# taohan10200/CRA5

Hardware: AMD Instinct MI355X
Metric: ERA5 frames/s (721x1440x268) encode+decode (higher is better)
Workload: dtype f32 (3xf16-split MFMA, fp32 accumulate)

## Files before the change

cra5_amd/csrc/attention_split_f16.hip:

```cpp
#include <hip/hip_runtime.h>
#include <math.h>
#include <stdlib.h>

#include "../../include/cra5_amd.h"
#include "split.h"

CRA5_RANGE_TU(attn)

typedef float f32x16 __attribute__((ext_vector_type(16)));
typedef _Float16 half8 __attribute__((ext_vector_type(8)));
typedef _Float16 half4 __attribute__((ext_vector_type(4)));
typedef __fp16 fp16x4 __attribute__((__vector_size__(4 * sizeof(__fp16))));
#if defined(__HIP_DEVICE_COMPILE__)
#define CRA5_TR_READ(P) \
  __builtin_bit_cast(half4, __builtin_amdgcn_ds_read_tr16_b64_v4f16((__attribute__((address_space(3))) fp16x4 *)(P)))
#else
#define CRA5_TR_READ(P) (*reinterpret_cast<const half4 *>(P))
#endif

namespace {

__device__ __forceinline__ int xcd_remap(int bid, int nb) {
  const int q = nb / 8, r = nb % 8;
  const int xcd = bid % 8, within = bid / 8;
  const int base = (xcd < r) ? xcd * (q + 1) : r * (q + 1) + (xcd - r) * q;
  return base + within;
}

struct WinGeom {
  int H, W, wh, ww, nwc;
};

__device__ __forceinline__ int token_of(const WinGeom &g, int wr, int wc, int t) {
  if (g.ww == g.W && g.wh == g.H) return t;
  const int r = t / g.ww, c = t - r * g.ww;
  const int gr = wr * g.wh + r, gc = wc * g.ww + c;
  return (gr < g.H && gc < g.W) ? gr * g.W + gc : -1;
}

#ifdef CRA5_ATTN_TRACE
__device__ unsigned long long g_attn_trace[6 * 8192];
#define CRA5_ATRACE(SLOT, VAL)                                                                          \
  if (threadIdx.x == 0 && atrace_idx < 8192) g_attn_trace[atrace_idx * 6 + (SLOT)] = (VAL);
#else
#define CRA5_ATRACE(SLOT, VAL)
#endif

constexpr int HD = 64;
constexpr int KS = 72;
constexpr int VS = 96;
constexpr int MAX_WIN_TOKENS = 1152;

struct BalArgs {
  int groups;
  int n_full;
  int n_wg_pass;
  int rem_tile0;
  int rem;
  int n_grp;
  int nkt;
  int maxp;
  float *ws;
};
__host__ __device__ __forceinline__ long bal_cut(long S, int G, int c) { return S * c / G; }
__host__ __device__ __forceinline__ int bal_piece_of(long S, int G, long s) {
  int c = (int)(s * G / S);
  if (c > G - 1) c = G - 1;
  while (c > 0 && bal_cut(S, G, c) > s) --c;
  while (c < G - 1 && bal_cut(S, G, c + 1) <= s) ++c;
  return c;
}
constexpr int WS_ROW = 68;

template <int NW, bool HI, bool GLOBAL, bool BAL = false, bool PLAIN = false>
__global__ __launch_bounds__(NW * 64, (NW >= 8 ? 1 : (NW == 4 ? 3 : 2))) void window_attention_split_kernel(
    const unsigned short *__restrict__ qkv, long ldq ,
    const unsigned short *__restrict__ pad_row, float *__restrict__ out, unsigned short *__restrict__ out_s,
    int Kp_out, int C, int heads, WinGeom g, int q_tiles , float scale, BalArgs bal) {
  static_assert(!BAL || GLOBAL, "the balanced schedule is for whole-grid launches");
  static_assert(!PLAIN || HI, "plain rows carry no lo plane");
  constexpr int NT = NW * 64;
  constexpr int PPR = PLAIN ? 8 : 16;
  constexpr int PIECES = 32 * PPR;
  constexpr int STG = (PIECES + NT - 1) / NT;

  constexpr int KPL = 32 * KS + 32;
  constexpr int VPL = 32 * VS;
  constexpr int KBUF = 2 * KPL, VBUF = 2 * VPL;
  __shared__ __attribute__((aligned(16))) unsigned short lds[2 * KBUF + 2 * VBUF];
  unsigned short *Ks = lds;
  unsigned short *Vt = lds + 2 * KBUF;
  constexpr int TAB = GLOBAL ? 1 : MAX_WIN_TOKENS;
  __shared__ long long tab[TAB];

  const int L = g.wh * g.ww;
  int head, win, n_seg = 1;
  int seg_tile0[2] = {0, 0}, seg_nact[2] = {NW, NW}, seg_j0[2] = {0, 0}, seg_j1[2] = {L / 32, L / 32}, seg_part[2] = {-1, -1};
  int seg_grp[2] = {0, 0};
  if (BAL) {
    const int pass = blockIdx.x / bal.n_wg_pass, w = blockIdx.x - pass * bal.n_wg_pass;
    int slot;
    if ((heads & 7) == 0 && (bal.n_wg_pass & 7) == 0) {
      const int xcd = w & 7, s_ = w >> 3;
      head = xcd * (heads >> 3) + s_ / bal.groups;
      slot = s_ % bal.groups;
    } else {
      head = w / bal.groups;
      slot = w % bal.groups;
    }
    win = 0;
    if (pass < bal.n_full) {
      seg_tile0[0] = (pass * bal.groups + slot) * NW;
    } else {
      const long S = (long)bal.n_grp * bal.nkt;
      const long s0 = bal_cut(S, bal.groups, slot), s1 = bal_cut(S, bal.groups, slot + 1);
      n_seg = 0;
      for (long s = s0; s < s1;) {
        const int gq = (int)(s / bal.nkt);
        const long e = min(s1, (long)(gq + 1) * bal.nkt);
        if (n_seg < 2) {
          seg_grp[n_seg] = gq;
          seg_tile0[n_seg] = bal.rem_tile0 + gq * NW;
          seg_nact[n_seg] = min(NW, bal.rem - gq * NW);
          seg_j0[n_seg] = (int)(s - (long)gq * bal.nkt);
          seg_j1[n_seg] = (int)(e - (long)gq * bal.nkt);
          seg_part[n_seg] = slot - bal_piece_of(S, bal.groups, (long)gq * bal.nkt);
          ++n_seg;
        }
        s = e;
      }
    }
  } else {
    const int pid = xcd_remap(blockIdx.x, gridDim.x);
    const int qt = pid % q_tiles;
    const int wh_id = pid / q_tiles;
    head = wh_id % heads;
    win = wh_id / heads;
    seg_tile0[0] = qt * NW;
  }
  const int wr = win / g.nwc, wc = win - wr * g.nwc;

  const int tid = threadIdx.x, lane = tid & 63, wave = tid >> 6;
  const int l31 = lane & 31, h = lane >> 5;
  const int hoff = head * HD;
  const long qoff = (PLAIN ? 1L : 2L) * hoff, koff = (PLAIN ? 1L : 2L) * (C + hoff), voff = (PLAIN ? 1L : 2L) * (2 * C + hoff);

  if (!GLOBAL) {
    const long long pad_delta = reinterpret_cast<const char *>(pad_row) - reinterpret_cast<const char *>(qkv);
    for (int t = tid; t < L; t += NT) {
      const int tok = token_of(g, wr, wc, t);
      tab[t] = (tok >= 0) ? (long long)tok * ldq * 2 : pad_delta;
    }
  }
  constexpr bool IDLE_SKIP = !GLOBAL || BAL;
  bool tab_ready = GLOBAL;
#pragma unroll 1
  for (int seg = 0; seg < n_seg; ++seg) {
  const int tile0 = seg_tile0[seg], n_active = seg_nact[seg], j0 = seg_j0[seg], j1 = seg_j1[seg];
#ifdef CRA5_ATTN_TRACE
  const int atrace_idx = GLOBAL ? 8192 : (int)blockIdx.x;
  const unsigned long long atrace_c0 = clock64();
#endif
  CRA5_ATRACE(0, wall_clock64());
  const int tq = (tile0 + wave) * 32 + l31;
  const int q_tok = (tq < L && wave < n_active) ? token_of(g, wr, wc, tq) : -1;
  const bool wave_active = __any(q_tok >= 0);
  if (!__syncthreads_or(wave_active ? 1 : 0)) continue;
  tab_ready = true;

  half8 qh[4], ql[4];
  {
    const unsigned short *qrow = ((q_tok >= 0) ? qkv + (size_t)q_tok * ldq : pad_row) + qoff;
#pragma unroll
    for (int s = 0; s < 4; ++s) {
      const int chunk = s >> 1, pp = 2 * (s & 1) + h;
      if (PLAIN) {
        qh[s] = *reinterpret_cast<const half8 *>(qrow + 16 * s + 8 * h);
        ql[s] = qh[s];
      } else {
        qh[s] = *reinterpret_cast<const half8 *>(qrow + chunk * 64 + pp * 8);
        ql[s] = *reinterpret_cast<const half8 *>(qrow + chunk * 64 + 32 + pp * 8);
      }
    }
  }
  const float cexp = scale * 1.44269504088896340736f;
  f32x16 negm;
#pragma unroll
  for (int r = 0; r < 16; ++r) negm[r] = 0.f;
  if (HI) {
#pragma unroll
    for (int s = 0; s < 4; ++s)
#pragma unroll
      for (int e = 0; e < 8; ++e) qh[s][e] = (_Float16)((float)qh[s][e] * cexp);
  }
  const float cmax = HI ? 1.0f : cexp;

  f32x16 o[2];
#pragma unroll
  for (int t = 0; t < 2; ++t)
#pragma unroll
    for (int r = 0; r < 16; ++r) o[t][r] = 0.f;
  float m_run = HI ? 0.f : -INFINITY, l_run = 0.f;

  const int n_tiles = j1 - j0;
  uint4 sk0 = make_uint4(0u, 0u, 0u, 0u), sk1 = sk0, sv0 = sk0, sv1 = sk0;
  static_assert(STG == 1 || STG == 2, "staging below is written out for one or two 16-byte pieces per thread");
  constexpr bool TWO = STG == 2;
  const int krow0 = min(tid / PPR, 31), krow1 = min((tid + NT) / PPR, 31);
  const long kcol = koff + (tid % PPR) * 8;
  const long vcol = voff + (tid % PPR) * 8;
  const unsigned short *kq0 = qkv + (size_t)(krow0 + 32 * j0) * ldq + kcol;
  const unsigned short *kq1 = qkv + (size_t)(krow1 + 32 * j0) * ldq + kcol;
  const unsigned short *vq0 = qkv + (size_t)(krow0 + 32 * j0) * ldq + vcol;
  const unsigned short *vq1 = qkv + (size_t)(krow1 + 32 * j0) * ldq + vcol;
  const long tile_step = 32 * ldq;
#define CRA5_ROW(JJ, ROW) \
  reinterpret_cast<const unsigned short *>(reinterpret_cast<const char *>(qkv) + tab[(JJ)*32 + (ROW)])
  const bool stage0 = (NT <= PIECES) || (tid < PIECES);
  const bool stage1 = TWO && (tid + NT < PIECES);
#define CRA5_K_LOAD(J)                                                                    \
  if (stage0) {                                                                           \
    if (GLOBAL) {                                                                         \
      sk0 = *reinterpret_cast<const uint4 *>(kq0);                                        \
      if (stage1) sk1 = *reinterpret_cast<const uint4 *>(kq1);                            \
      const long st_ = ((J) < n_tiles - 1) ? tile_step : 0;  \
      kq0 += st_;                                                                         \
      kq1 += st_;                                                                         \
    } else {                                                                              \
      const int jj_ = min((J), n_tiles - 1);                                              \
      sk0 = *reinterpret_cast<const uint4 *>(CRA5_ROW(jj_, krow0) + kcol);                \
      if (stage1) sk1 = *reinterpret_cast<const uint4 *>(CRA5_ROW(jj_, krow1) + kcol);    \
    }                                                                                     \
  }
#define CRA5_V_LOAD(J)                                                                    \
  if (stage0) {                                                                           \
    if (GLOBAL) {                                                                         \
      sv0 = *reinterpret_cast<const uint4 *>(vq0);                                        \
      if (stage1) sv1 = *reinterpret_cast<const uint4 *>(vq1);                            \
      const long st_ = ((J) < n_tiles - 1) ? tile_step : 0;                               \
      vq0 += st_;                                                                         \
      vq1 += st_;                                                                         \
    } else {                                                                              \
      const int jj_ = min((J), n_tiles - 1);                                              \
      sv0 = *reinterpret_cast<const uint4 *>(CRA5_ROW(jj_, krow0) + vcol);                \
      if (stage1) sv1 = *reinterpret_cast<const uint4 *>(CRA5_ROW(jj_, krow1) + vcol);    \
    }                                                                                     \
  }
#define CRA5_K_STORE1(P, BUF)                                                             \
  {                                                                                       \
    const int idx = tid + (P)*NT;                                                         \
    if (idx < PIECES) {                                                                   \
      const int row = idx / PPR, piece = idx % PPR;                                       \
      const int plane = PLAIN ? 0 : (piece >> 2) & 1, d0 = PLAIN ? 8 * piece : 32 * (piece >> 3) + 8 * (piece & 3); \
      *reinterpret_cast<uint4 *>(Ks + (BUF)*KBUF + plane * KPL + row * KS + d0) = sk##P;  \
    }                                                                                     \
  }
#define CRA5_K_STORE(BUF) { CRA5_K_STORE1(0, BUF) if (TWO) CRA5_K_STORE1(1, BUF) }
#define CRA5_V_STORE1(P, BUF)                                                             \
  {                                                                                       \
    const int idx = tid + (P)*NT;                                                         \
    if (idx < PIECES) {                                                                   \
      const int row = idx / PPR, piece = idx % PPR;                                       \
      const int plane = PLAIN ? 0 : (piece >> 2) & 1, d0 = PLAIN ? 8 * piece : 32 * (piece >> 3) + 8 * (piece & 3); \
      *reinterpret_cast<uint4 *>(Vt + (BUF)*VBUF + plane * VPL + row * VS + d0) = sv##P;  \
    }                                                                                     \
  }
#define CRA5_V_STORE(BUF) { CRA5_V_STORE1(0, BUF) if (TWO) CRA5_V_STORE1(1, BUF) }
#define CRA5_SCORES(DST, KB)                                                              \
  {                                                                                       \
    f32x16 acc_;                                                                          \
    _Pragma("unroll") for (int r = 0; r < 16; ++r) acc_[r] = 0.f;                         \
    _Pragma("unroll") for (int st = 0; st < 4; ++st) {                                    \
      const half8 kh = *reinterpret_cast<const half8 *>(k_base + (KB)*KBUF + 16 * st);     \
      const half8 kl = *reinterpret_cast<const half8 *>(k_base + (KB)*KBUF + KPL + 16 * st); \
      if (!HI) {                                                                          \
        acc_ = __builtin_amdgcn_mfma_f32_32x32x16_f16(kl, qh[st], acc_, 0, 0, 0);         \
        acc_ = __builtin_amdgcn_mfma_f32_32x32x16_f16(kh, ql[st], acc_, 0, 0, 0);         \
      }                                                                                   \
      if (HI && st == 0) {                                                                \
        CRA5_MFMA_FROM(acc_, kh, qh[0], negm);                                            \
      } else {                                                                            \
        acc_ = __builtin_amdgcn_mfma_f32_32x32x16_f16(kh, qh[st], acc_, 0, 0, 0);         \
      }                                                                                   \
    }                                                                                     \
    DST = acc_;                                                                           \
  }
#if defined(__HIP_DEVICE_COMPILE__)
#define CRA5_MFMA_FROM(D, A, B, C) \
  asm("s_nop 3\n\tv_mfma_f32_32x32x16_f16 %0, %1, %2, %3" : "=&v"(D) : "v"(A), "v"(B), "v"(C))
#else
#define CRA5_MFMA_FROM(D, A, B, C) (D) = (C)
#endif

  const unsigned short *k_base = Ks + l31 * KS + 8 * h;
  const unsigned short *v_base = Vt + (4 * h + ((lane & 15) >> 2)) * VS + 16 * ((lane >> 4) & 1) + 4 * (lane & 3);

#if defined(__HIP_DEVICE_COMPILE__)
#define CRA5_XHALF_MAX(X)                                                                 \
  ({                                                                                      \
    float a_ = (X), b_ = (X), r_;                                                         \
    asm("s_nop 1\n\tv_permlane32_swap_b32_e32 %0, %1\n\ts_nop 1\n\tv_max_f32_e32 %2, %0, %1" \
        : "+v"(a_), "+v"(b_), "=v"(r_));                                                  \
    r_;                                                                                   \
  })
#define CRA5_MAX2_VALU(A, B)                                                              \
  ({                                                                                      \
    float r_;                                                                             \
    asm("v_max_f32_e32 %0, %1, %2" : "=v"(r_) : "v"(A), "v"(B));                          \
    r_;                                                                                   \
  })
#else
#define CRA5_XHALF_MAX(X) (X)
#define CRA5_MAX2_VALU(A, B) fmaxf((A), (B))
#endif
#if !defined(__HIP_DEVICE_COMPILE__)
#define CRA5_TILE_MAX(S)                                                                  \
  ({                                                                                      \
    float m_ = fmaxf(fmaxf(fmaxf(S[0], S[1]), fmaxf(S[2], S[3])), fmaxf(fmaxf(S[4], S[5]), fmaxf(S[6], S[7]))); \
    float n_ = fmaxf(fmaxf(fmaxf(S[8], S[9]), fmaxf(S[10], S[11])), fmaxf(fmaxf(S[12], S[13]), fmaxf(S[14], S[15]))); \
    CRA5_XHALF_MAX(fmaxf(m_, n_)) * cmax;       \
  })
#else
#define CRA5_MAX3(A, B, C) fmaxf(fmaxf((A), (B)), (C))
#define CRA5_TILE_MAX(S)                                                                  \
  ({                                                                                      \
    const float a_ = CRA5_MAX3(S[0], S[1], S[2]), b_ = CRA5_MAX3(S[3], S[4], S[5]), c_ = CRA5_MAX3(S[6], S[7], S[8]); \
    const float d_ = CRA5_MAX3(S[9], S[10], S[11]), e_ = CRA5_MAX3(S[12], S[13], S[14]);     \
    const float f_ = CRA5_MAX3(a_, b_, c_), g_ = CRA5_MAX3(d_, e_, S[15]);                   \
    CRA5_XHALF_MAX(CRA5_MAX2_VALU(f_, g_)) * cmax;  \
  })
#endif

  f32x16 s_cur;
  CRA5_K_LOAD(0);
  CRA5_V_LOAD(0);
  CRA5_K_STORE(0);
  CRA5_V_STORE(0);
  CRA5_K_LOAD(1);
  CRA5_K_STORE(1);
  __syncthreads();
  CRA5_K_LOAD(2);
  CRA5_V_LOAD(1);
  CRA5_SCORES(s_cur, 0);
  float mloc = CRA5_TILE_MAX(s_cur);
  __syncthreads();

  auto key_tile = [&](const int j, f32x16 &s_cur, f32x16 &s_next) __attribute__((always_inline)) {
    const int kb = (j + 1) & 1, vb = j & 1;
    if (!IDLE_SKIP || wave_active) {
    constexpr float DEFER_LOG2 = 8.0f;
    auto shift = [&](float delta, const bool rescale, f32x16 *also) __attribute__((always_inline)) {
      delta = (float)(_Float16)fminf(fmaxf(delta, -60000.f), 60000.f);
      if (rescale) {
        const float alpha = __builtin_amdgcn_exp2f(-delta);
        l_run *= alpha;
#pragma unroll
        for (int t = 0; t < 2; ++t)
#pragma unroll
          for (int r = 0; r < 16; ++r) o[t][r] *= alpha;
      }
      m_run += delta;
      half8 e0, bd;
#pragma unroll
      for (int e = 0; e < 8; ++e) {
        e0[e] = (_Float16)0.0f;
        bd[e] = (_Float16)0.0f;
      }
      e0[0] = (_Float16)(h == 0 ? 1.0f : 0.0f);
      bd[0] = (_Float16)(h == 0 ? -delta : 0.0f);
      s_cur = __builtin_amdgcn_mfma_f32_32x32x16_f16(e0, bd, s_cur, 0, 0, 0);
      negm = __builtin_amdgcn_mfma_f32_32x32x16_f16(e0, bd, negm, 0, 0, 0);
      if (also) *also = __builtin_amdgcn_mfma_f32_32x32x16_f16(e0, bd, *also, 0, 0, 0);
#if defined(__HIP_DEVICE_COMPILE__)
      asm volatile("s_nop 15\n\ts_nop 3" ::: "memory");
#endif
    };
    if (HI) {
      if (j == 0) shift(mloc, false, nullptr);
    } else if (!__all(mloc - m_run <= DEFER_LOG2)) {
      const float m_new = fmaxf(m_run, mloc);
      const float alpha = __builtin_amdgcn_exp2f(m_run - m_new);
      l_run *= alpha;
#pragma unroll
      for (int t = 0; t < 2; ++t)
#pragma unroll
        for (int r = 0; r < 16; ++r) o[t][r] *= alpha;
      m_run = m_new;
    }
    const float m_new = m_run;
#if defined(__HIP_DEVICE_COMPILE__)
    if (!HI) {
#define CRA5_FENCE() __builtin_amdgcn_sched_barrier(0)
#define CRA5_STAGE(MFMA_STMT) \
  CRA5_FENCE();               \
  MFMA_STMT;                  \
  CRA5_FENCE();
#define CRA5_KFRAG(PLANE, ST) (*reinterpret_cast<const half8 *>(k_base + kb * KBUF + (PLANE)*KPL + 16 * (ST)))
#define CRA5_MM(A, B, C) __builtin_amdgcn_mfma_f32_32x32x16_f16((A), (B), (C), 0, 0, 0)
      typedef _Float16 half2v __attribute__((ext_vector_type(2)));
      typedef unsigned u32x4 __attribute__((ext_vector_type(4)));
      float p[16], psum = 0.f;
      u32x4 phw[2], plw[2];
      auto exp_half = [&](const int u) __attribute__((always_inline)) {
        p[2 * u] = __builtin_amdgcn_exp2f(fmaf(s_cur[2 * u], cexp, -m_new));
        p[2 * u + 1] = __builtin_amdgcn_exp2f(fmaf(s_cur[2 * u + 1], cexp, -m_new));
      };
      auto split_half = [&](const int u) __attribute__((always_inline)) {
        const int r = 2 * u;
        const half2v h2 = {(_Float16)p[r], (_Float16)p[r + 1]};
        const unsigned hh = __builtin_bit_cast(unsigned, h2);
        float d0, d1;
        asm("v_fma_mix_f32 %0, %2, -1.0, %3 op_sel_hi:[1,0,0]\n\t"
            "v_fma_mix_f32 %1, %2, -1.0, %4 op_sel:[1,0,0] op_sel_hi:[1,0,0]"
            : "=&v"(d0), "=&v"(d1) : "v"(hh), "v"(p[r]), "v"(p[r + 1]));
        psum += p[r];
        psum += p[r + 1];
        const half2v l2 = {(_Float16)d0, (_Float16)d1};
        unsigned ll = __builtin_bit_cast(unsigned, l2);
        asm("" : "+v"(ll));
        phw[u >> 2][u & 3] = hh;
        plw[u >> 2][u & 3] = ll;
      };
#define ph(T) __builtin_bit_cast(half8, phw[T])
#define pl(T) __builtin_bit_cast(half8, plw[T])
      half8 vh[2], vl[2];
      auto v_frag = [&](const int t, const int plane, const int dt) __attribute__((always_inline)) {
        const unsigned short *vp = v_base + vb * VBUF + plane * VPL + 16 * t * VS + 32 * dt;
        const half4 a0 = CRA5_TR_READ(vp);
        const half4 a1 = CRA5_TR_READ(vp + 8 * VS);
        return __builtin_shufflevector(a0, a1, 0, 1, 2, 3, 4, 5, 6, 7);
      };
      half8 kh0 = CRA5_KFRAG(0, 0), kl0 = CRA5_KFRAG(1, 0), kh1 = CRA5_KFRAG(0, 1), kl1 = CRA5_KFRAG(1, 1);
      f32x16 acc;
#pragma unroll
      for (int r = 0; r < 16; ++r) acc[r] = 0.f;
      CRA5_STAGE(acc = CRA5_MM(kl0, qh[0], acc))
      exp_half(0);
      CRA5_STAGE(acc = CRA5_MM(kh0, ql[0], acc))
      exp_half(1);
      CRA5_STAGE(acc = CRA5_MM(kh0, qh[0], acc))
      split_half(0);
      const half8 kh2 = CRA5_KFRAG(0, 2), kl2 = CRA5_KFRAG(1, 2);
      CRA5_STAGE(acc = CRA5_MM(kl1, qh[1], acc))
      exp_half(2);
      CRA5_STAGE(acc = CRA5_MM(kh1, ql[1], acc))
      split_half(1);
      CRA5_STAGE(acc = CRA5_MM(kh1, qh[1], acc))
      exp_half(3);
      const half8 kh3 = CRA5_KFRAG(0, 3), kl3 = CRA5_KFRAG(1, 3);
      CRA5_STAGE(acc = CRA5_MM(kl2, qh[2], acc))
      split_half(2);
      CRA5_STAGE(acc = CRA5_MM(kh2, ql[2], acc))
      exp_half(4);
      CRA5_STAGE(acc = CRA5_MM(kh2, qh[2], acc))
      split_half(3);
      CRA5_STAGE(acc = CRA5_MM(kl3, qh[3], acc))
      exp_half(5);
      vl[0] = v_frag(0, 1, 0);
      vl[1] = v_frag(0, 1, 1);
      CRA5_STAGE(acc = CRA5_MM(kh3, ql[3], acc))
      split_half(4);
      CRA5_STAGE(acc = CRA5_MM(kh3, qh[3], acc))
      split_half(5);
      vh[0] = v_frag(0, 0, 0);
      vh[1] = v_frag(0, 0, 1);
      s_next = acc;
      CRA5_STAGE(o[0] = CRA5_MM(vl[0], ph(0), o[0]))
      exp_half(6);
      CRA5_STAGE(o[1] = CRA5_MM(vl[1], ph(0), o[1]))
      exp_half(7);
      CRA5_STAGE(o[0] = CRA5_MM(vh[0], pl(0), o[0]))
      split_half(6);
      CRA5_STAGE(o[1] = CRA5_MM(vh[1], pl(0), o[1]))
      split_half(7);
      vl[0] = v_frag(1, 1, 0);
      vl[1] = v_frag(1, 1, 1);
      CRA5_STAGE(o[0] = CRA5_MM(vh[0], ph(0), o[0]))
      l_run += psum;
      CRA5_STAGE(o[1] = CRA5_MM(vh[1], ph(0), o[1]))
      vh[0] = v_frag(1, 0, 0);
      vh[1] = v_frag(1, 0, 1);
      CRA5_STAGE(o[0] = CRA5_MM(vl[0], ph(1), o[0]))
      const float ma = CRA5_MAX3(s_next[0], s_next[1], s_next[2]), mb = CRA5_MAX3(s_next[3], s_next[4], s_next[5]);
      const float mc = CRA5_MAX3(s_next[6], s_next[7], s_next[8]), md = CRA5_MAX3(s_next[9], s_next[10], s_next[11]);
      const float me = CRA5_MAX3(s_next[12], s_next[13], s_next[14]);
      CRA5_STAGE(o[1] = CRA5_MM(vl[1], ph(1), o[1]))
      const float mf = CRA5_MAX3(ma, mb, mc), mg = CRA5_MAX3(md, me, s_next[15]);
      const float mfg = CRA5_MAX2_VALU(mf, mg);
      CRA5_STAGE(o[0] = CRA5_MM(vh[0], pl(1), o[0]))
      const float mx = CRA5_XHALF_MAX(mfg);
      CRA5_STAGE(o[1] = CRA5_MM(vh[1], pl(1), o[1]))
      mloc = mx * cmax;
      CRA5_STAGE(o[0] = CRA5_MM(vh[0], ph(1), o[0]))
      CRA5_STAGE(o[1] = CRA5_MM(vh[1], ph(1), o[1]))
#undef ph
#undef pl
#undef CRA5_MM
#undef CRA5_KFRAG
#undef CRA5_STAGE
#undef CRA5_FENCE
    } else
#endif
    {
    CRA5_SCORES(s_next, kb);
    float psum = 0.f;
    half8 ph[2], pl[2];
#if defined(__HIP_DEVICE_COMPILE__)
    if (HI) {
      typedef _Float16 half2v __attribute__((ext_vector_type(2)));
      typedef _Float16 half8v __attribute__((ext_vector_type(8)));
      const half2v ones = {(_Float16)1.0f, (_Float16)1.0f};
      auto exps = [&]() __attribute__((always_inline)) {
        psum = 0.f;
#pragma unroll
        for (int t = 0; t < 2; ++t) {
          half2v hp[4];
#pragma unroll
          for (int i = 0; i < 4; ++i) {
            hp[i] = half2v{(_Float16)__builtin_amdgcn_exp2f(s_cur[8 * t + 2 * i]), (_Float16)__builtin_amdgcn_exp2f(s_cur[8 * t + 2 * i + 1])};
            psum = __builtin_amdgcn_fdot2(hp[i], ones, psum, false);
          }
          ph[t] = half8v{hp[0][0], hp[0][1], hp[1][0], hp[1][1], hp[2][0], hp[2][1], hp[3][0], hp[3][1]};
        }
      };
      exps();
      constexpr float P_SAFE = 8192.0f;
      if (!__all(psum <= P_SAFE)) {
        const float mrel = CRA5_TILE_MAX(s_cur);
        shift(fmaxf(mrel, 0.f), true, &s_next);
        exps();
      }
#pragma unroll
      for (int t = 0; t < 2; ++t)
#pragma unroll
        for (int e = 0; e < 8; ++e) pl[t][e] = (_Float16)0.0f;
    }
#else
#pragma unroll
    for (int r = 0; r < 16; ++r) {
      const float p = HI ? (float)(_Float16)__builtin_amdgcn_exp2f(s_cur[r]) : __builtin_amdgcn_exp2f(fmaf(s_cur[r], cexp, -m_new));
      psum += p;
      const _Float16 hi = (_Float16)p;
      const _Float16 lo = (_Float16)(p - (float)hi);
      ph[r >> 3][r & 7] = hi;
      pl[r >> 3][r & 7] = lo;
    }
#endif
    l_run += psum;
#pragma unroll
    for (int t = 0; t < 2; ++t) {
      half8 vh[2], vl[2];
#pragma unroll
      for (int dt = 0; dt < 2; ++dt) {
        const unsigned short *vp = v_base + vb * VBUF + 16 * t * VS + 32 * dt;
        const unsigned short *vq = vp + VPL;
        const half4 a0 = CRA5_TR_READ(vp);
        const half4 a1 = CRA5_TR_READ(vp + 8 * VS);
        const half4 b0 = CRA5_TR_READ(vq);
        const half4 b1 = CRA5_TR_READ(vq + 8 * VS);
        vh[dt] = __builtin_shufflevector(a0, a1, 0, 1, 2, 3, 4, 5, 6, 7);
        vl[dt] = __builtin_shufflevector(b0, b1, 0, 1, 2, 3, 4, 5, 6, 7);
      }
      if (!HI) {
        o[0] = __builtin_amdgcn_mfma_f32_32x32x16_f16(vl[0], ph[t], o[0], 0, 0, 0);
        o[1] = __builtin_amdgcn_mfma_f32_32x32x16_f16(vl[1], ph[t], o[1], 0, 0, 0);
        o[0] = __builtin_amdgcn_mfma_f32_32x32x16_f16(vh[0], pl[t], o[0], 0, 0, 0);
        o[1] = __builtin_amdgcn_mfma_f32_32x32x16_f16(vh[1], pl[t], o[1], 0, 0, 0);
      }
      o[0] = __builtin_amdgcn_mfma_f32_32x32x16_f16(vh[0], ph[t], o[0], 0, 0, 0);
      o[1] = __builtin_amdgcn_mfma_f32_32x32x16_f16(vh[1], ph[t], o[1], 0, 0, 0);
    }
    if (!HI) mloc = CRA5_TILE_MAX(s_next);
    }
    }
    CRA5_K_STORE(j & 1);
    CRA5_V_STORE((j + 1) & 1);
    CRA5_K_LOAD(j + 3);
    CRA5_V_LOAD(j + 2);
    __syncthreads();
  };
  CRA5_ATRACE(1, wall_clock64());
  f32x16 s_alt;
  const int n_loop = n_tiles;
  int jt = 0;
  for (; jt + 1 < n_loop; jt += 2) {
    key_tile(jt, s_cur, s_alt);
    key_tile(jt + 1, s_alt, s_cur);
  }
  if (jt < n_loop) key_tile(jt, s_cur, s_alt);
  CRA5_ATRACE(2, wall_clock64());
  CRA5_ATRACE(4, (unsigned long long)n_tiles);

  const float l_tot = l_run + __shfl_xor(l_run, 32, 64);
  if (BAL && seg_part[seg] >= 0) {
    if (q_tok >= 0) {
      float *wrow = bal.ws + (((((size_t)head * bal.n_grp + seg_grp[seg]) * bal.maxp + seg_part[seg]) * NW + wave) * 32 + l31) * WS_ROW;
#pragma unroll
      for (int t = 0; t < 2; ++t)
#pragma unroll
        for (int gq = 0; gq < 4; ++gq) {
          const int d = 32 * t + 8 * gq + 4 * h;
          *reinterpret_cast<float4 *>(wrow + d) = make_float4(o[t][4 * gq + 0], o[t][4 * gq + 1], o[t][4 * gq + 2], o[t][4 * gq + 3]);
        }
      if (h == 0) {
        wrow[64] = m_run;
        wrow[65] = l_tot;
      }
    }
    continue;
  }
  {
    const bool live = q_tok >= 0;
    const float inv = live ? 1.0f / l_tot : 0.0f;
    float *orow = (out && live) ? out + (size_t)q_tok * C + hoff : nullptr;
    unsigned short *srow = (out_s && live) ? out_s + (size_t)q_tok * 2 * Kp_out : nullptr;
#pragma unroll
    for (int t = 0; t < 2; ++t)
#pragma unroll
      for (int pr = 0; pr < 2; ++pr) {
        float va[4], vb[4];
#pragma unroll
        for (int k = 0; k < 4; ++k) {
          va[k] = o[t][4 * (2 * pr) + k] * inv;
          vb[k] = o[t][4 * (2 * pr + 1) + k] * inv;
        }
        if (orow) {
          *reinterpret_cast<float4 *>(orow + 32 * t + 16 * pr + 4 * h) = make_float4(va[0], va[1], va[2], va[3]);
          *reinterpret_cast<float4 *>(orow + 32 * t + 16 * pr + 8 + 4 * h) = make_float4(vb[0], vb[1], vb[2], vb[3]);
        }
        if (out_s) {
          unsigned ha0, la0, ha1, la1, hb0, lb0, hb1, lb1;
          cra5_split_pair(va[0], va[1], ha0, la0);
          cra5_split_pair(va[2], va[3], ha1, la1);
          cra5_split_pair(vb[0], vb[1], hb0, lb0);
          cra5_split_pair(vb[2], vb[3], hb1, lb1);
#if defined(__HIP_DEVICE_COMPILE__)
#define CRA5_SWAP32(A, B)                                                  \
  {                                                                        \
    const auto r_ = __builtin_amdgcn_permlane32_swap((A), (B), false, false); \
    (A) = r_[0];                                                           \
    (B) = r_[1];                                                           \
  }
          CRA5_SWAP32(ha0, hb0);
          CRA5_SWAP32(ha1, hb1);
          CRA5_SWAP32(la0, lb0);
          CRA5_SWAP32(la1, lb1);
#undef CRA5_SWAP32
#endif
          if (srow) {
            const int c0 = hoff + 32 * t + 16 * pr + 8 * h;
            unsigned short *sp = srow + (PLAIN ? c0 : (c0 >> 5) * 64 + (c0 & 31));
            *reinterpret_cast<uint4 *>(sp) = make_uint4(ha0, ha1, hb0, hb1);
            if (!HI) *reinterpret_cast<uint4 *>(sp + 32) = make_uint4(la0, la1, lb0, lb1);
          }
        }
      }
  }
  CRA5_ATRACE(3, wall_clock64());
  CRA5_ATRACE(5, clock64() - atrace_c0);
  }
  (void)tab_ready;
}

__global__ __launch_bounds__(256) void attention_merge_kernel(const float *__restrict__ ws, float *__restrict__ out,
                                                              unsigned short *__restrict__ out_s, int Kp_out, int C,
                                                              BalArgs bal, int nw, int plain) {
  const int t = blockIdx.x % nw, hg = blockIdx.x / nw;
  const int grp = hg % bal.n_grp, head = hg / bal.n_grp;
  if (grp * nw + t >= bal.rem) return;
  const long S = (long)bal.n_grp * bal.nkt;
  const int c0 = bal_piece_of(S, bal.groups, (long)grp * bal.nkt);
  const int c1 = bal_piece_of(S, bal.groups, (long)(grp + 1) * bal.nkt - 1);
  const int np = c1 - c0 + 1;
  const int q = threadIdx.x >> 3, d0 = (threadIdx.x & 7) * 8;
  const size_t pstride = (size_t)nw * 32 * WS_ROW;
  const float *base = ws + ((((size_t)head * bal.n_grp + grp) * bal.maxp) * nw + t) * 32 * WS_ROW + (size_t)q * WS_ROW;
  float M = -INFINITY;
  for (int c = 0; c < np; ++c) M = fmaxf(M, base[c * pstride + 64]);
  float acc[8] = {0.f, 0.f, 0.f, 0.f, 0.f, 0.f, 0.f, 0.f}, lsum = 0.f;
  for (int c = 0; c < np; ++c) {
    const float *r = base + c * pstride;
    const float a = __builtin_amdgcn_exp2f(r[64] - M);
    lsum = fmaf(r[65], a, lsum);
    const float4 v0 = *reinterpret_cast<const float4 *>(r + d0), v1 = *reinterpret_cast<const float4 *>(r + d0 + 4);
    acc[0] = fmaf(v0.x, a, acc[0]);
    acc[1] = fmaf(v0.y, a, acc[1]);
    acc[2] = fmaf(v0.z, a, acc[2]);
    acc[3] = fmaf(v0.w, a, acc[3]);
    acc[4] = fmaf(v1.x, a, acc[4]);
    acc[5] = fmaf(v1.y, a, acc[5]);
    acc[6] = fmaf(v1.z, a, acc[6]);
    acc[7] = fmaf(v1.w, a, acc[7]);
  }
  const float inv = 1.0f / lsum;
  const int tok = (bal.rem_tile0 + grp * nw + t) * 32 + q, col = head * HD + d0;
#pragma unroll
  for (int k = 0; k < 8; ++k) acc[k] *= inv;
  if (out) {
    *reinterpret_cast<float4 *>(out + (size_t)tok * C + col) = make_float4(acc[0], acc[1], acc[2], acc[3]);
    *reinterpret_cast<float4 *>(out + (size_t)tok * C + col + 4) = make_float4(acc[4], acc[5], acc[6], acc[7]);
  }
  if (out_s) {
    unsigned short *srow = out_s + (size_t)tok * 2 * Kp_out;
    if (plain) {
      cra5_store_plain4(srow, col, acc[0], acc[1], acc[2], acc[3]);
      cra5_store_plain4(srow, col + 4, acc[4], acc[5], acc[6], acc[7]);
    } else {
      cra5_store_split4(srow, col, acc[0], acc[1], acc[2], acc[3]);
      cra5_store_split4(srow, col + 4, acc[4], acc[5], acc[6], acc[7]);
    }
  }
}

int cu_count() {
  static const int n = [] {
    int dev = 0, v = 0;
    if (hipGetDevice(&dev) != hipSuccess) return 256;
    if (hipDeviceGetAttribute(&v, hipDeviceAttributeMultiprocessorCount, dev) != hipSuccess || v <= 0) return 256;
    return v;
  }();
  return n;
}

constexpr int NW_GLOBAL = 12;

bool balanced_plan(int L, int heads, BalArgs &b) {
  const int P = cu_count(), T = L / 32;
  if (P % heads) return false;
  b.groups = P / heads;
  b.n_full = T / (b.groups * NW_GLOBAL);
  b.rem_tile0 = b.n_full * b.groups * NW_GLOBAL;
  b.rem = T - b.rem_tile0;
  b.n_grp = (b.rem + NW_GLOBAL - 1) / NW_GLOBAL;
  b.nkt = T;
  b.n_wg_pass = heads * b.groups;
  b.ws = nullptr;
  b.maxp = 0;
  const long S = (long)b.n_grp * b.nkt;
  for (int g = 0; g < b.n_grp; ++g) {
    const int np = bal_piece_of(S, b.groups, (long)(g + 1) * b.nkt - 1) - bal_piece_of(S, b.groups, (long)g * b.nkt) + 1;
    if (np > b.maxp) b.maxp = np;
  }
  if (!(b.n_full >= 1 && (b.rem == 0 || (b.n_grp <= b.groups && S >= b.groups)))) return false;
  for (int c = 0; b.rem && c < b.groups; ++c) {
    const long s0 = bal_cut(S, b.groups, c), s1 = bal_cut(S, b.groups, c + 1);
    if (s1 > s0 && (s1 - 1) / b.nkt - s0 / b.nkt + 1 > 2) return false;
  }
  return true;
}

size_t balanced_ws_bytes(const BalArgs &b, int heads) {
  return (size_t)heads * b.n_grp * b.maxp * NW_GLOBAL * 32 * WS_ROW * sizeof(float);
}

template <bool HI, bool PLAIN = false>
int launch_balanced(const unsigned short *qkv, long ldq, const unsigned short *pad_row, float *out, unsigned short *out_s,
                    int Kp_out, int C, int heads, int H, int W, float scale, BalArgs b, float *ws, hipStream_t st) {
  WinGeom g;
  g.H = H;
  g.W = W;
  g.wh = H;
  g.ww = W;
  g.nwc = 1;
  b.ws = ws;
  const int n_pass = b.n_full + (b.rem ? 1 : 0);
  hipLaunchKernelGGL((window_attention_split_kernel<NW_GLOBAL, HI, true, true, PLAIN>), dim3(n_pass * b.n_wg_pass),
                     dim3(NW_GLOBAL * 64), 0, st, qkv, ldq, pad_row, out, out_s, Kp_out, C, heads, g, 0, scale, b);
  int rc = (int)hipGetLastError();
  if (rc || b.rem == 0) return rc;
  hipLaunchKernelGGL(attention_merge_kernel, dim3(heads * b.n_grp * NW_GLOBAL), dim3(256), 0, st, ws, out, out_s, Kp_out,
                     C, b, NW_GLOBAL, PLAIN ? 1 : 0);
  return (int)hipGetLastError();
}

template <int NW, bool HI, bool GLOBAL, bool PLAIN = false>
int launch(const unsigned short *qkv, long ldq, const unsigned short *pad_row, float *out, unsigned short *out_s,
           int Kp_out, int C, int heads, int H, int W, int wh, int ww, float scale, hipStream_t st) {
  WinGeom g;
  g.H = H;
  g.W = W;
  g.wh = wh;
  g.ww = ww;
  const int nwr = (H + wh - 1) / wh;
  g.nwc = (W + ww - 1) / ww;
  const int L = wh * ww;
  const int q_tiles = (L + NW * 32 - 1) / (NW * 32);
  hipLaunchKernelGGL((window_attention_split_kernel<NW, HI, GLOBAL, false, PLAIN>), dim3(q_tiles * nwr * g.nwc * heads), dim3(NW * 64), 0, st,
                     qkv, ldq, pad_row, out, out_s, Kp_out, C, heads, g, q_tiles, scale, BalArgs{});
  return (int)hipGetLastError();
}

}

static int attention_dispatch(const uint16_t *qkv_split, int qkv_kp, const uint16_t *pad_row_split, float *out,
                              uint16_t *out_split, int out_kp, int C, int heads, int H, int W, int wh, int ww,
                              float scale, int hi_only, void *workspace, size_t workspace_bytes, void *stream,
                              bool want_balanced) {
  if (!qkv_split || !pad_row_split || (!out && !out_split) || heads <= 0 || C % heads) return CRA5_ERR_ARG;
  if (C / heads != 64 || qkv_kp != 3 * C) return CRA5_ERR_ARG;
  if (wh <= 0 || ww <= 0 || H <= 0 || W <= 0 || (wh * ww) % 32) return CRA5_ERR_ARG;
  if (out_split && (out_kp < C || out_kp % 32)) return CRA5_ERR_ARG;
  if (((uintptr_t)qkv_split & 15) || ((uintptr_t)pad_row_split & 15)) return CRA5_ERR_ARG;
  hipStream_t st = (hipStream_t)stream;
  const int L = wh * ww;
  if (hi_only != 0 && hi_only != 1 && hi_only != 3) return CRA5_ERR_ARG;
  const bool plain = hi_only == 3;
  const long ldq = 2L * qkv_kp;
  const bool whole = (wh == H && ww == W);
  if (!whole && L > MAX_WIN_TOKENS) return CRA5_ERR_ARG;
#define CRA5_ATT_GO(NWV, HIV, GLV) \
  return launch<NWV, HIV, GLV>(qkv_split, ldq, pad_row_split, out, out_split, out_kp, C, heads, H, W, wh, ww, scale, st)
  if (whole) {
    BalArgs b;
    if (want_balanced && balanced_plan(L, heads, b) &&
        (balanced_ws_bytes(b, heads) == 0 ||
         (workspace && ((uintptr_t)workspace & 15) == 0 && workspace_bytes >= balanced_ws_bytes(b, heads)))) {
      float *ws = reinterpret_cast<float *>(workspace);
      if (plain)
        return launch_balanced<true, true>(qkv_split, ldq, pad_row_split, out, out_split, out_kp, C, heads, H, W, scale, b, ws, st);
      if (hi_only)
        return launch_balanced<true>(qkv_split, ldq, pad_row_split, out, out_split, out_kp, C, heads, H, W, scale, b, ws, st);
      return launch_balanced<false>(qkv_split, ldq, pad_row_split, out, out_split, out_kp, C, heads, H, W, scale, b, ws, st);
    }
    if (plain) return launch<NW_GLOBAL, true, true, true>(qkv_split, ldq, pad_row_split, out, out_split, out_kp, C, heads, H, W, wh, ww, scale, st);
    if (hi_only) CRA5_ATT_GO(NW_GLOBAL, true, true);
    CRA5_ATT_GO(NW_GLOBAL, false, true);
  }
  if (plain) return launch<4, true, false, true>(qkv_split, ldq, pad_row_split, out, out_split, out_kp, C, heads, H, W, wh, ww, scale, st);
  if (hi_only) CRA5_ATT_GO(4, true, false);
  CRA5_ATT_GO(4, false, false);
#undef CRA5_ATT_GO
}

#ifdef CRA5_ATTN_TRACE
extern "C" int cra5_debug_attn_trace(unsigned long long *host, int n_rows) {
  if (n_rows < 1 || n_rows > 8192) return CRA5_ERR_ARG;
  if (hipDeviceSynchronize() != hipSuccess) return CRA5_ERR_ARG;
  int rc = (int)hipMemcpyFromSymbol(host, HIP_SYMBOL(g_attn_trace), sizeof(unsigned long long) * 6 * n_rows);
  void *p = nullptr;
  if (hipGetSymbolAddress(&p, HIP_SYMBOL(g_attn_trace)) == hipSuccess) hipMemset(p, 0, sizeof(unsigned long long) * 6 * 8192);
  return rc;
}
#endif

extern "C" int cra5_window_attention_split(const uint16_t *qkv_split, int qkv_kp, const uint16_t *pad_row_split,
                                           float *out, uint16_t *out_split, int out_kp, int C, int heads, int H,
                                           int W, int wh, int ww, float scale, int hi_only, void *stream) {
  return attention_dispatch(qkv_split, qkv_kp, pad_row_split, out, out_split, out_kp, C, heads, H, W, wh, ww, scale,
                            hi_only, nullptr, 0, stream, false);
}

extern "C" size_t cra5_attention_workspace_bytes(int n_tokens, int heads) {
  BalArgs b;
  if (n_tokens <= 0 || heads <= 0 || (n_tokens % 32) || !balanced_plan(n_tokens, heads, b)) return 0;
  return balanced_ws_bytes(b, heads);
}

extern "C" int cra5_window_attention_split_ws(const uint16_t *qkv_split, int qkv_kp, const uint16_t *pad_row_split,
                                              float *out, uint16_t *out_split, int out_kp, int C, int heads, int H,
                                              int W, int wh, int ww, float scale, int hi_only, void *workspace,
                                              size_t workspace_bytes, void *stream) {
  return attention_dispatch(qkv_split, qkv_kp, pad_row_split, out, out_split, out_kp, C, heads, H, W, wh, ww, scale,
                            hi_only, workspace, workspace_bytes, stream, true);
}

extern "C" int cra5_attention_balanced_plan(int n_tokens, int heads, size_t *workspace_bytes) {
  BalArgs b;
  if (workspace_bytes) *workspace_bytes = 0;
  if (n_tokens <= 0 || heads <= 0 || (n_tokens % 32) || !balanced_plan(n_tokens, heads, b)) return 0;
  if (workspace_bytes) *workspace_bytes = balanced_ws_bytes(b, heads);
  return 1;
}
```

Before: 31.99.

## Triple-buffer K tiles in LDS for global attention and prefetch K fragments

For the global-window attention path, the K staging buffer goes from a double buffer to a three-slot ring in LDS, so global loads run one tile further ahead. The first K fragments for the next tile are read into registers during the previous tile's PV MFMAs, which hides LDS read latency at the start of the score computation. Debug-only per-wave timing counters are also added behind the trace macro. The cost is extra LDS per block, which could reduce occupancy, and more registers held for the prefetched fragments.

```diff
diff --git a/cra5_amd/csrc/attention_split_f16.hip b/cra5_amd/csrc/attention_split_f16.hip
--- a/cra5_amd/csrc/attention_split_f16.hip
+++ b/cra5_amd/csrc/attention_split_f16.hip
@@ -42,8 +42,13 @@
 __device__ unsigned long long g_attn_trace[6 * 8192];
 #define CRA5_ATRACE(SLOT, VAL)                                                                          \
   if (threadIdx.x == 0 && atrace_idx < 8192) g_attn_trace[atrace_idx * 6 + (SLOT)] = (VAL);
+__device__ unsigned long long g_attn_ktrace[5 * 16384];
+#define CRA5_KTRACE_DECL unsigned long long ktr_a = 0, ktr_b = 0, ktr_c = 0, ktr_stage = 0, ktr_wait = 0, ktr_first = 0, ktr_loop0 = 0;
+#define CRA5_KTRACE(...) if (GLOBAL) { __VA_ARGS__ }
 #else
 #define CRA5_ATRACE(SLOT, VAL)
+#define CRA5_KTRACE_DECL
+#define CRA5_KTRACE(...)
 #endif
 
 constexpr int HD = 64;
@@ -87,9 +92,10 @@
   constexpr int KPL = 32 * KS + 32;
   constexpr int VPL = 32 * VS;
   constexpr int KBUF = 2 * KPL, VBUF = 2 * VPL;
-  __shared__ __attribute__((aligned(16))) unsigned short lds[2 * KBUF + 2 * VBUF];
+  constexpr int KRING = GLOBAL ? 3 : 2;
+  __shared__ __attribute__((aligned(16))) unsigned short lds[KRING * KBUF + 2 * VBUF];
   unsigned short *Ks = lds;
-  unsigned short *Vt = lds + 2 * KBUF;
+  unsigned short *Vt = lds + KRING * KBUF;
   constexpr int TAB = GLOBAL ? 1 : MAX_WIN_TOKENS;
   __shared__ long long tab[TAB];
 
@@ -246,16 +252,18 @@
       if (stage1) sv1 = *reinterpret_cast<const uint4 *>(CRA5_ROW(jj_, krow1) + vcol);    \
     }                                                                                     \
   }
-#define CRA5_K_STORE1(P, BUF)                                                             \
+#define CRA5_K_STORE1(P, OFF)                                                             \
   {                                                                                       \
     const int idx = tid + (P)*NT;                                                         \
     if (idx < PIECES) {                                                                   \
       const int row = idx / PPR, piece = idx % PPR;                                       \
       const int plane = PLAIN ? 0 : (piece >> 2) & 1, d0 = PLAIN ? 8 * piece : 32 * (piece >> 3) + 8 * (piece & 3); \
-      *reinterpret_cast<uint4 *>(Ks + (BUF)*KBUF + plane * KPL + row * KS + d0) = sk##P;  \
+      *reinterpret_cast<uint4 *>(Ks + (OFF) + plane * KPL + row * KS + d0) = sk##P;       \
     }                                                                                     \
   }
-#define CRA5_K_STORE(BUF) { CRA5_K_STORE1(0, BUF) if (TWO) CRA5_K_STORE1(1, BUF) }
+#define CRA5_K_STORE_AT(OFF) { CRA5_K_STORE1(0, OFF) if (TWO) CRA5_K_STORE1(1, OFF) }
+#define CRA5_K_STORE(BUF) CRA5_K_STORE_AT((BUF)*KBUF)
+#define CRA5_RING_NEXT(OFF) ((OFF) == 2 * KBUF ? 0 : (OFF) + KBUF)
 #define CRA5_V_STORE1(P, BUF)                                                             \
   {                                                                                       \
     const int idx = tid + (P)*NT;                                                         \
@@ -266,13 +274,13 @@
     }                                                                                     \
   }
 #define CRA5_V_STORE(BUF) { CRA5_V_STORE1(0, BUF) if (TWO) CRA5_V_STORE1(1, BUF) }
-#define CRA5_SCORES(DST, KB)                                                              \
+#define CRA5_SCORES(DST, KP)                                                              \
   {                                                                                       \
     f32x16 acc_;                                                                          \
     _Pragma("unroll") for (int r = 0; r < 16; ++r) acc_[r] = 0.f;                         \
     _Pragma("unroll") for (int st = 0; st < 4; ++st) {                                    \
-      const half8 kh = *reinterpret_cast<const half8 *>(k_base + (KB)*KBUF + 16 * st);     \
-      const half8 kl = *reinterpret_cast<const half8 *>(k_base + (KB)*KBUF + KPL + 16 * st); \
+      const half8 kh = *reinterpret_cast<const half8 *>((KP) + 16 * st);                  \
+      const half8 kl = *reinterpret_cast<const half8 *>((KP) + KPL + 16 * st);            \
       if (!HI) {                                                                          \
         acc_ = __builtin_amdgcn_mfma_f32_32x32x16_f16(kl, qh[st], acc_, 0, 0, 0);         \
         acc_ = __builtin_amdgcn_mfma_f32_32x32x16_f16(kh, ql[st], acc_, 0, 0, 0);         \
@@ -332,19 +340,40 @@
 #endif
 
   f32x16 s_cur;
+  const unsigned short *kring_rd = k_base + KBUF;
+  int kring_ph = 1, kring_st = 0;
+  half8 kf[4];
+#define CRA5_RING_ADVANCE()                                                               \
+  {                                                                                       \
+    kring_rd += (kring_ph == 2) ? -2 * KBUF : KBUF;                                       \
+    kring_ph = (kring_ph == 2) ? 0 : kring_ph + 1;                                        \
+  }
+#define CRA5_KF_READ()                                                                    \
+  {                                                                                       \
+    kf[0] = *reinterpret_cast<const half8 *>(kring_rd);                                   \
+    kf[1] = *reinterpret_cast<const half8 *>(kring_rd + KPL);                             \
+    kf[2] = *reinterpret_cast<const half8 *>(kring_rd + 16);                              \
+    kf[3] = *reinterpret_cast<const half8 *>(kring_rd + KPL + 16);                        \
+  }
   CRA5_K_LOAD(0);
   CRA5_V_LOAD(0);
   CRA5_K_STORE(0);
   CRA5_V_STORE(0);
   CRA5_K_LOAD(1);
   CRA5_K_STORE(1);
+  if (KRING == 3) {
+    CRA5_K_LOAD(2);
+    CRA5_K_STORE(2);
+  }
   __syncthreads();
-  CRA5_K_LOAD(2);
+  CRA5_K_LOAD(KRING);
   CRA5_V_LOAD(1);
-  CRA5_SCORES(s_cur, 0);
+  CRA5_SCORES(s_cur, k_base);
   float mloc = CRA5_TILE_MAX(s_cur);
+  if (KRING == 3 && !HI) CRA5_KF_READ();
   __syncthreads();
 
+  CRA5_KTRACE_DECL
   auto key_tile = [&](const int j, f32x16 &s_cur, f32x16 &s_next) __attribute__((always_inline)) {
     const int kb = (j + 1) & 1, vb = j & 1;
     if (!IDLE_SKIP || wave_active) {
@@ -395,7 +424,8 @@
   CRA5_FENCE();               \
   MFMA_STMT;                  \
   CRA5_FENCE();
-#define CRA5_KFRAG(PLANE, ST) (*reinterpret_cast<const half8 *>(k_base + kb * KBUF + (PLANE)*KPL + 16 * (ST)))
+      const unsigned short *kp = (KRING == 3) ? kring_rd : k_base + kb * KBUF;
+#define CRA5_KFRAG(PLANE, ST) (*reinterpret_cast<const half8 *>(kp + (PLANE)*KPL + 16 * (ST)))
 #define CRA5_MM(A, B, C) __builtin_amdgcn_mfma_f32_32x32x16_f16((A), (B), (C), 0, 0, 0)
       typedef _Float16 half2v __attribute__((ext_vector_type(2)));
       typedef unsigned u32x4 __attribute__((ext_vector_type(4)));
@@ -430,11 +460,17 @@
         const half4 a1 = CRA5_TR_READ(vp + 8 * VS);
         return __builtin_shufflevector(a0, a1, 0, 1, 2, 3, 4, 5, 6, 7);
       };
-      half8 kh0 = CRA5_KFRAG(0, 0), kl0 = CRA5_KFRAG(1, 0), kh1 = CRA5_KFRAG(0, 1), kl1 = CRA5_KFRAG(1, 1);
+      half8 kh0, kl0, kh1, kl1;
+      if (KRING == 3) {
+        kh0 = kf[0], kl0 = kf[1], kh1 = kf[2], kl1 = kf[3];
+      } else {
+        kh0 = CRA5_KFRAG(0, 0), kl0 = CRA5_KFRAG(1, 0), kh1 = CRA5_KFRAG(0, 1), kl1 = CRA5_KFRAG(1, 1);
+      }
       f32x16 acc;
 #pragma unroll
       for (int r = 0; r < 16; ++r) acc[r] = 0.f;
       CRA5_STAGE(acc = CRA5_MM(kl0, qh[0], acc))
+      CRA5_KTRACE(ktr_first += clock64() - ktr_c;)
       exp_half(0);
       CRA5_STAGE(acc = CRA5_MM(kh0, ql[0], acc))
       exp_half(1);
@@ -477,6 +513,7 @@
       vl[1] = v_frag(1, 1, 1);
       CRA5_STAGE(o[0] = CRA5_MM(vh[0], ph(0), o[0]))
       l_run += psum;
+      if (KRING == 3) CRA5_RING_ADVANCE();
       CRA5_STAGE(o[1] = CRA5_MM(vh[1], ph(0), o[1]))
       vh[0] = v_frag(1, 0, 0);
       vh[1] = v_frag(1, 0, 1);
@@ -491,7 +528,15 @@
       const float mx = CRA5_XHALF_MAX(mfg);
       CRA5_STAGE(o[1] = CRA5_MM(vh[1], pl(1), o[1]))
       mloc = mx * cmax;
+      if (KRING == 3) {
+        kf[0] = *reinterpret_cast<const half8 *>(kring_rd);
+        kf[1] = *reinterpret_cast<const half8 *>(kring_rd + KPL);
+      }
       CRA5_STAGE(o[0] = CRA5_MM(vh[0], ph(1), o[0]))
+      if (KRING == 3) {
+        kf[2] = *reinterpret_cast<const half8 *>(kring_rd + 16);
+        kf[3] = *reinterpret_cast<const half8 *>(kring_rd + KPL + 16);
+      }
       CRA5_STAGE(o[1] = CRA5_MM(vh[1], ph(1), o[1]))
 #undef ph
 #undef pl
@@ -502,7 +547,12 @@
     } else
 #endif
     {
-    CRA5_SCORES(s_next, kb);
+    if (KRING == 3) {
+      CRA5_SCORES(s_next, kring_rd);
+      CRA5_RING_ADVANCE();
+    } else {
+      CRA5_SCORES(s_next, k_base + kb * KBUF);
+    }
     float psum = 0.f;
     half8 ph[2], pl[2];
 #if defined(__HIP_DEVICE_COMPILE__)
@@ -573,13 +623,22 @@
     if (!HI) mloc = CRA5_TILE_MAX(s_next);
     }
     }
-    CRA5_K_STORE(j & 1);
+    CRA5_KTRACE(ktr_a = clock64();)
+    if (KRING == 3) {
+      CRA5_K_STORE_AT(kring_st);
+      kring_st = CRA5_RING_NEXT(kring_st);
+    } else {
+      CRA5_K_STORE(j & 1);
+    }
     CRA5_V_STORE((j + 1) & 1);
-    CRA5_K_LOAD(j + 3);
+    CRA5_K_LOAD(j + KRING + 1);
     CRA5_V_LOAD(j + 2);
+    CRA5_KTRACE(ktr_b = clock64();)
     __syncthreads();
+    CRA5_KTRACE(ktr_c = clock64(); ktr_stage += ktr_b - ktr_a; ktr_wait += ktr_c - ktr_b;)
   };
   CRA5_ATRACE(1, wall_clock64());
+  CRA5_KTRACE(ktr_c = ktr_loop0 = clock64();)
   f32x16 s_alt;
   const int n_loop = n_tiles;
   int jt = 0;
@@ -590,6 +649,10 @@
   if (jt < n_loop) key_tile(jt, s_cur, s_alt);
   CRA5_ATRACE(2, wall_clock64());
   CRA5_ATRACE(4, (unsigned long long)n_tiles);
+  CRA5_KTRACE(if (GLOBAL && seg == 0 && lane == 0 && (blockIdx.x * NW + wave) < 16384) {
+    unsigned long long *kt_ = g_attn_ktrace + (size_t)(blockIdx.x * NW + wave) * 5;
+    kt_[0] = ktr_stage, kt_[1] = ktr_wait, kt_[2] = ktr_first, kt_[3] = (unsigned long long)n_tiles, kt_[4] = clock64() - ktr_loop0;
+  })
 
   const float l_tot = l_run + __shfl_xor(l_run, 32, 64);
   if (BAL && seg_part[seg] >= 0) {
@@ -833,6 +896,15 @@
 }
 
 #ifdef CRA5_ATTN_TRACE
+extern "C" int cra5_debug_attn_ktrace(unsigned long long *host, int n_rows) {
+  if (n_rows < 1 || n_rows > 16384) return CRA5_ERR_ARG;
+  if (hipDeviceSynchronize() != hipSuccess) return CRA5_ERR_ARG;
+  int rc = (int)hipMemcpyFromSymbol(host, HIP_SYMBOL(g_attn_ktrace), sizeof(unsigned long long) * 5 * n_rows);
+  void *p = nullptr;
+  if (hipGetSymbolAddress(&p, HIP_SYMBOL(g_attn_ktrace)) == hipSuccess) (void)hipMemset(p, 0, sizeof(unsigned long long) * 5 * 16384);
+  return rc;
+}
+
 extern "C" int cra5_debug_attn_trace(unsigned long long *host, int n_rows) {
   if (n_rows < 1 || n_rows > 8192) return CRA5_ERR_ARG;
   if (hipDeviceSynchronize() != hipSuccess) return CRA5_ERR_ARG;
```

Result: no change. 32.19, median of 6 (+0.6%).
